# byungsook/neural-flow-style

Measured on AMD Instinct MI355X. Metric: stylization iters/sec on 200^3 smoke grid, 8 views, higher is better.
Workload: dtype f32 (3xbf16 split-limb MFMA, f32 accumulate)

## Files before the change

neural-flow-style_amd/_lib.py:

```python
from __future__ import annotations

import ctypes as C
import os
import subprocess

_HERE = os.path.dirname(os.path.abspath(__file__))
LIB_PATH = os.environ.get("NFS_LIB_PATH") or os.path.join(_HERE, "libnfs_hip.so")
CSRC_DIR = os.path.join(_HERE, "csrc")


class NfsLibraryError(RuntimeError):
    pass


NFS_EINVAL, NFS_ELAUNCH = -1, -2


class NfsError(RuntimeError):

    def __init__(self, name, code, msg):
        RuntimeError.__init__(self, "%s failed (%d): %s" % (name, code, msg))
        self.name, self.code = name, int(code)


# ... 111 lines not shown
    "nfs_gram_style_group_workspace_floats": [_P, _I],
    "nfs_gram_style_group_parts": [_P, _I],
    "nfs_gram_style_group_fwd": [_P, _I, _P, _P, _L, _P],
    "nfs_gram_group_bwd": [_P, _I, _P],
    "nfs_hist_loss_masked": [_P, _P, _P, _P, _P, _I, _I, _I, _I, _I, _F, _I, _P],
    "nfs_hist_loss_wide_workspace_floats": [_I, _I, _I, _I],
    "nfs_hist_loss_wide": [_P, _P, _P, _P, _P, _P, _L, _I, _I, _I, _I, _I, _F, _I, _P],
    "nfs_resize_bicubic_tf1": [_P, _P, _I, _I, _I, _I, _I, _I, _P],
    "nfs_style_mask_apply": [_P, _P, _P, _P, _I, _I, _I, _P],
    "nfs_style_mask_bwd": [_P, _P, _P, _P, _I, _I, _I, _P],
    "nfs_tv_loss": [_P, _P, _P, _I, _I, _I, _I, _F, _P],
    "nfs_p2g_fwd": [_P, _P, _P, _P, _P, _I, _I, C.POINTER(SplatCfg), _P],
    "nfs_p2g_bwd": [_P, _P, _P, _P, _P, _P, _P, _P, _I, _I, C.POINTER(SplatCfg), _P],
    "nfs_p2g_wavg_finish": [_P, _P, _P, _L, _I, _F, _P],
    "nfs_p2g_wavg_finish_bwd": [_P, _P, _P, _P, _P, _L, _I, _F, _P],
    "nfs_p2g_wavg_bwd": [_P, _P, _P, _P, _P, _P, _P, _I, _I, _F, C.POINTER(SplatCfg), _P],
    "nfs_g2p_fwd": [_P, _P, _P, _I, _I, _I, _I, _I, _L, _I, _P],
    "nfs_adam_tf_step": [_P, _P, _P, _P, _L, _F, _F, _F, _F, _P],
    "nfs_fill": [_P, _F, _L, _P],
    "nfs_axpy": [_P, _P, _F, _L, _P],
    "nfs_slab_pack": [_P, _P, _I, _L, _I, _I, _P],
    "nfs_colour_clamp_gather": [_P, _P, _P, _L, _I, _P],
    "nfs_clamp01_bwd": [_P, _P, _P, _L, _P],
    "nfs_colour_clamp_scatter_bwd": [_P, _P, _P, _P, _L, _I, _P],
    "nfs_iterate_update": [_P, _P, _L, _P],
}
_RESTYPE = {"nfs_last_error": C.c_char_p, "nfs_conv3x3_packed_floats": C.c_int64,
            "nfs_conv3x3_workspace_floats": C.c_int64, "nfs_gram_workspace_floats": C.c_int64,
            "nfs_conv3x3_relu_bits_words": C.c_int64, "nfs_gram_style_group_workspace_floats": C.c_int64, "nfs_hist_loss_wide_workspace_floats": C.c_int64,
            "nfs_conv3x3_executed_flops": C.c_double, "nfs_conv2d_packed_floats": C.c_int64,
            "nfs_conv2d_workspace_floats": C.c_int64, "nfs_conv2d_group_workspace_floats": C.c_int64}

_lib = None
ABI_VERSION = 152


def build(verbose=False):
    jobs = os.environ.get("MAX_JOBS") or str(min(os.cpu_count() or 4, 16))
    r = subprocess.run(["make", "-C", CSRC_DIR, "-j", jobs],
                       capture_output=True, text=True)
    if verbose or r.returncode != 0:
        print(r.stdout[-4000:], r.stderr[-4000:])
    if r.returncode != 0:
        raise NfsLibraryError("building libnfs_hip.so failed")
    return LIB_PATH


def lib():
    global _lib
    if _lib is None:
        if not os.path.exists(LIB_PATH):
            raise NfsLibraryError(
                "libnfs_hip.so is missing (%s): run `python -c 'import __graft_entry__ as g; g.build()'` "
                "-- there is no CPU fallback for the product path" % LIB_PATH)
        import torch
        try:
            L = C.CDLL(LIB_PATH)
        except OSError as e:
            raise NfsLibraryError("cannot load %s: %s" % (LIB_PATH, e))
        for name, argt in SIGNATURES.items():
            try:
                f = getattr(L, name)
            except AttributeError:
                raise NfsLibraryError("libnfs_hip.so does not export %s (stale build?)" % name)
            f.argtypes = argt
            f.restype = _RESTYPE.get(name, C.c_int)
        if L.nfs_version() < ABI_VERSION:
# ... 24 lines not shown
```

neural-flow-style_amd/csrc/api.hip:

```cpp
#include "common.h"

namespace nfs {
static thread_local char g_err[512] = "";
void set_error(const char* fmt, ...) {
  va_list ap;
  va_start(ap, fmt);
  vsnprintf(g_err, sizeof(g_err), fmt, ap);
  va_end(ap);
}
}

extern "C" {
int nfs_version(void) { return 152; }
const char* nfs_last_error(void) { return nfs::g_err; }
int nfs_device_cus(void) {
  int dev = 0;
  hipDeviceProp_t p;
  if (hipGetDevice(&dev) != hipSuccess || hipGetDeviceProperties(&p, dev) != hipSuccess) {
    nfs::set_error("nfs_device_cus: no HIP device");
    return NFS_ELAUNCH;
  }
  return p.multiProcessorCount;
}
}
```

neural-flow-style_amd/csrc/vgg.hip:

```cpp
#include "common.h"

#include <mutex>
#include <stdlib.h>

namespace nfs {

int64_t winograd_workspace_floats(int B, int H, int W, int K, int N);
int64_t winograd_packed_floats(int Ci, int Co);
int winograd_path(int B, int H, int W, int K, int N);
int winograd_tile();
int64_t winograd5_bits_words(int B, int H, int W, int C);
int winograd_pack(const float* w_hwio, float* up, int Ci, int Co, int kind, hipStream_t s);
int winograd_conv(const float* x, const float* U, const float* aux0, const float* aux1, float* y, float* ws, int B,
                  int H, int W, int K, int N, int mode, int relu, int cus, hipStream_t s, float* ypool,
                  const float* xmask, uint32_t* in_bits, uint32_t* out_bits, bool pooled_grad);
static inline bool winograd_eligible(int K, int N) {
  static const int min_ch = [] { const char* e = getenv("NFS_WINOGRAD_MIN_CH"); return e ? atoi(e) : 64; }();
  return K >= min_ch && N >= min_ch && K % 32 == 0 && N % 64 == 0;
}

typedef float f32x16 __attribute__((ext_vector_type(16)));

constexpr int KC = 32;
constexpr int LDS_STRIDE = 36;
constexpr int BM = 128;
constexpr int PATCH_MAX = 192;

struct ConvArgs {
  const float* x;
  const float* wp;
  const float* aux0;
  const float* aux1;
  float* y;
  float* ws;
  int B, H, W, Kc, Nc;
  int TH, TW, tiles_c;
  int relu, ksplit;
  int dbg;
};

template <int MODE>
__device__ __forceinline__ float conv_epilogue(const ConvArgs& a, float v, int n, int64_t idx) {
// ... 564 lines not shown
  return (int64_t)9 * Ci * Co + (winograd_eligible(K, N) ? winograd_packed_floats(Ci, Co) : 0);
}

int nfs_conv3x3_pack(const float* w_hwio, float* packed, int Ci, int Co, int kind, nfs_stream_t stream) {
  NFS_REQUIRE(w_hwio && packed, "nfs_conv3x3_pack: null pointer");
  NFS_REQUIRE(kind == 0 || kind == 1, "nfs_conv3x3_pack: kind must be 0 or 1");
  NFS_REQUIRE(Ci == 3 || (Ci % 64 == 0), "nfs_conv3x3_pack: Ci must be 3 or a multiple of 64");
  NFS_REQUIRE(Co % 64 == 0, "nfs_conv3x3_pack: Co must be a multiple of 64");
  const int64_t n = (int64_t)9 * Ci * Co;
  hipLaunchKernelGGL(pack_kernel, dim3(blocks_for(n, 256)), dim3(256), 0, as_stream(stream), w_hwio, packed, Ci, Co,
                     kind);
  const int K = kind == 0 ? Ci : Co, N = kind == 0 ? Co : Ci;
  if (winograd_eligible(K, N))
    if (int e = winograd_pack(w_hwio, packed + n, Ci, Co, kind, as_stream(stream))) return e;
  return check_launch("nfs_conv3x3_pack");
}

int64_t nfs_conv3x3_workspace_floats(int B, int H, int W, int Ci, int Co) {
  if (B <= 0 || H <= 0 || W <= 0 || Ci <= 0 || Co <= 0) return 0;
  if (winograd_eligible(Ci, Co) && winograd_eligible(Co, Ci) && H >= 2 && W >= 2)
    return winograd_workspace_floats(B, H, W, Ci > Co ? Ci : Co, Ci > Co ? Ci : Co);
  const int64_t n = Ci > Co ? Ci : Co;
  const int64_t want = (int64_t)16 * B * H * W * n;
  return want < ((int64_t)32 << 20) ? want : ((int64_t)32 << 20);
}

int64_t nfs_conv3x3_relu_bits_words(int B, int H, int W, int Ci, int Co, int pooled) {
  if (B <= 0 || H < 2 || W < 2 || Ci <= 0 || Co <= 0 || Ci % 64 || Co % 64) return 0;
  static const bool off = getenv("NFS_NO_RELU_BITS") != nullptr;
  ConvArgs a{nullptr, nullptr, nullptr, nullptr, nullptr, nullptr, B, H, W, Ci, Co, 0, 0, 0, 1, 1, 0};
  float dummy = 0.f;
  if (off || !takes_fused_pool(a, &dummy, INT64_MAX)) return 0;
  if (!pooled && winograd_path(B, H, W, Ci, Co) == 2) return winograd5_bits_words(B, H, W, Ci);
  const int64_t T = (int64_t)B * ((H + 3) / 4) * ((W + 3) / 4);
  return T * (Ci / 2) + (pooled ? T * (Co / 2) : 0);
}

double nfs_conv3x3_executed_flops(int B, int H, int W, int K, int N, int pooled) {
  if (B <= 0 || H <= 0 || W <= 0 || K <= 0 || N <= 0) return 0.0;
  static const bool no_wg = getenv("NFS_NO_WINOGRAD") != nullptr;
  const double direct = 2.0 * B * H * W * 9.0 * K * N;
  if (no_wg || !winograd_eligible(K, N) || H < 2 || W < 2) return direct;
  const int m = winograd_tile();
  if (m == 4 && !pooled && winograd_path(B, H, W, K, N) == 2)
    return 2.0 * 49.0 * B * ((H + 4) / 5) * ((W + 4) / 5) * (double)K * N;
  return 2.0 * (m + 2) * (m + 2) * B * ((H + m - 1) / m) * ((W + m - 1) / m) * (double)K * N;
}

static inline uint32_t* out_bits_of(uint32_t* relu_bits, int B, int H, int W, int Ci) {
  return relu_bits ? relu_bits + (int64_t)B * ((H + 3) / 4) * ((W + 3) / 4) * (Ci / 2) : nullptr;
}

int nfs_conv3x3_fwd(const float* x, const float* packed_fwd, const float* bias, float* y, int B, int H, int W, int Ci,
                    int Co, int relu, float* workspace, int64_t workspace_floats, uint32_t* relu_bits,
                    nfs_stream_t stream) {
  NFS_REQUIRE(x && packed_fwd && y, "nfs_conv3x3_fwd: null pointer");
  NFS_REQUIRE(B > 0 && H > 0 && W > 0, "nfs_conv3x3_fwd: non-positive dimension");
  NFS_REQUIRE((int64_t)B * H * W < ((int64_t)1 << 31) / 4, "nfs_conv3x3_fwd: too many pixels");
  NFS_REQUIRE(Co > 0 && Co % 64 == 0, "nfs_conv3x3_fwd: Co must be a multiple of 64");
  static const bool old_c3 = getenv("NFS_C3_OLD") != nullptr;
  if (Ci == 3 && Co == 64 && !old_c3) {
    const int tiles_x = (W + C3F_TW - 1) / C3F_TW, tiles_y = (H + C3F_TH - 1) / C3F_TH;
    static const int per_cu = [] { const char* e = getenv("NFS_C3F_BLOCKS"); return e ? atoi(e) : 4; }();
    const int64_t ntiles = (int64_t)B * tiles_x * tiles_y, cap = 256 * (int64_t)per_cu;
    hipLaunchKernelGGL(conv3x3_c3co64_fwd_kernel, dim3((unsigned)(per_cu > 0 && ntiles > cap ? cap : ntiles)), dim3(256), 0,
                       as_stream(stream), x, packed_fwd, bias, y, B, H, W, relu, tiles_x, tiles_y);
    return check_launch("nfs_conv3x3_fwd(c3, Co=64, MFMA)");
  }
  if (Ci == 3) {
    const int64_t n = (int64_t)B * H * W * (Co / 4);
    hipLaunchKernelGGL(conv3x3_c3_fwd_kernel, dim3(blocks_for(n, 256)), dim3(256), 27 * Co * sizeof(float),
                       as_stream(stream), x, packed_fwd, bias, y, B, H, W, Co, relu);
    return check_launch("nfs_conv3x3_fwd(c3)");
  }
  NFS_REQUIRE(Ci > 0 && Ci % 32 == 0, "nfs_conv3x3_fwd: Ci must be 3 or a multiple of 32");
  ConvArgs a{x, packed_fwd, bias, nullptr, y, nullptr, B, H, W, Ci, Co, 0, 0, 0, relu, 1, 0};
  return launch_conv<0>(a, workspace, workspace_floats, as_stream(stream), nullptr, nullptr, relu_bits, nullptr);
}

int nfs_conv3x3_dgrad(const float* gy, const float* packed_dgrad, const float* x_in, const float* addend, float* gx,
                      int B, int H, int W, int Ci, int Co, float* workspace, int64_t workspace_floats,
                      const uint32_t* relu_bits, int addend_unmasked, nfs_stream_t stream) {
  NFS_REQUIRE(gy && packed_dgrad && gx, "nfs_conv3x3_dgrad: null pointer");
  NFS_REQUIRE(B > 0 && H > 0 && W > 0, "nfs_conv3x3_dgrad: non-positive dimension");
  NFS_REQUIRE((int64_t)B * H * W < ((int64_t)1 << 31) / 4, "nfs_conv3x3_dgrad: too many pixels");
  NFS_REQUIRE(Co > 0 && Co % 32 == 0, "nfs_conv3x3_dgrad: Co must be a multiple of 32");
  if (Ci == 3) {
    NFS_REQUIRE(!x_in && !addend, "nfs_conv3x3_dgrad: Ci=3 takes no mask/addend");
    static const bool old_c3 = getenv("NFS_C3_OLD") != nullptr;
    if (Co == 64 && !old_c3) {
      const int tiles_x = (W + C3D_TW - 1) / C3D_TW, tiles_y = (H + C3D_TH - 1) / C3D_TH;
      static const int per_cu = [] { const char* e = getenv("NFS_C3D_BLOCKS"); return e ? atoi(e) : 2; }();
      const int64_t ntiles = (int64_t)B * tiles_x * tiles_y, cap = 256 * (int64_t)per_cu;
      hipLaunchKernelGGL(conv3x3_c3co64_dgrad_kernel, dim3((unsigned)(per_cu > 0 && ntiles > cap ? cap : ntiles)),
                         dim3(256), 0, as_stream(stream), gy, packed_dgrad, gx, B, H, W, tiles_x, tiles_y);
      return check_launch("nfs_conv3x3_dgrad(c3, Co=64, MFMA)");
    }
    const int64_t n = (int64_t)B * H * W;
    hipLaunchKernelGGL(conv3x3_c3_dgrad_kernel, dim3(blocks_for(n, 256)), dim3(256), 27 * Co * sizeof(float),
                       as_stream(stream), gy, packed_dgrad, gx, B, H, W, Co);
    return check_launch("nfs_conv3x3_dgrad(c3)");
  }
  NFS_REQUIRE(Ci > 0 && Ci % 64 == 0, "nfs_conv3x3_dgrad: Ci must be 3 or a multiple of 64");
  ConvArgs a{gy, packed_dgrad, x_in, addend, gx, nullptr, B, H, W, Co, Ci, 0, 0, 0, addend_unmasked ? 1 : 0, 1, 0};
  NFS_REQUIRE(!addend_unmasked || (x_in && takes_fused_pool(a, workspace, workspace_floats)),
              "nfs_conv3x3_dgrad: addend_unmasked needs x_in and the F(4x4) Winograd path");
  return launch_conv<1>(a, workspace, workspace_floats, as_stream(stream), nullptr, nullptr,
                        const_cast<uint32_t*>(relu_bits), nullptr);
}

int nfs_conv3x3_fwd_pool(const float* x, const float* packed_fwd, const float* bias, float* y, float* y_pool, int B, int H,
                         int W, int Ci, int Co, int relu, float* workspace, int64_t workspace_floats,
                         uint32_t* relu_bits, nfs_stream_t stream) {
  NFS_REQUIRE(x && packed_fwd && y_pool, "nfs_conv3x3_fwd_pool: null pointer");
  NFS_REQUIRE(B > 0 && H > 1 && W > 1, "nfs_conv3x3_fwd_pool: need H, W >= 2");
  NFS_REQUIRE((int64_t)B * H * W < ((int64_t)1 << 31) / 4, "nfs_conv3x3_fwd_pool: too many pixels");
  NFS_REQUIRE(Co > 0 && Co % 64 == 0 && Ci > 0 && Ci % 32 == 0, "nfs_conv3x3_fwd_pool: Ci %% 32, Co %% 64 required");
  ConvArgs a{x, packed_fwd, bias, nullptr, y, nullptr, B, H, W, Ci, Co, 0, 0, 0, relu, 1, 0};
  if (takes_fused_pool(a, workspace, workspace_floats)) {
    NFS_REQUIRE(y || relu_bits, "nfs_conv3x3_fwd_pool: without y the ReLU bit cache must be recorded");
    return launch_conv<0>(a, workspace, workspace_floats, as_stream(stream), y_pool, nullptr, relu_bits,
                          out_bits_of(relu_bits, B, H, W, Ci));
  }
  NFS_REQUIRE(!relu_bits, "nfs_conv3x3_fwd_pool: the ReLU bit cache needs the fused Winograd path "
                          "(nfs_conv3x3_relu_bits_words returned 0 for this layer)");
  NFS_REQUIRE(y, "nfs_conv3x3_fwd_pool: y may only be NULL on the fused Winograd path with a ReLU bit cache");
  if (int e = launch_conv<0>(a, workspace, workspace_floats, as_stream(stream))) return e;
  return nfs_avgpool2_fwd(y, y_pool, B, H, W, Co, stream);
}

int nfs_conv3x3_dgrad_pool(const float* gy_pool, const float* x_out, const float* packed_dgrad, const float* x_in,
                           const float* addend, float* gx, int B, int H, int W, int Ci, int Co, float* workspace,
                           int64_t workspace_floats, const uint32_t* relu_bits, int addend_unmasked,
                           nfs_stream_t stream) {
  NFS_REQUIRE(gy_pool && packed_dgrad && gx, "nfs_conv3x3_dgrad_pool: null pointer");
  NFS_REQUIRE(x_out || relu_bits, "nfs_conv3x3_dgrad_pool: x_out or the layer's ReLU bit cache is required");
  NFS_REQUIRE(B > 0 && H > 1 && W > 1, "nfs_conv3x3_dgrad_pool: need H, W >= 2");
  NFS_REQUIRE((int64_t)B * H * W < ((int64_t)1 << 31) / 4, "nfs_conv3x3_dgrad_pool: too many pixels");
  NFS_REQUIRE(Co > 0 && Co % 32 == 0 && Ci > 0 && Ci % 64 == 0, "nfs_conv3x3_dgrad_pool: Co %% 32, Ci %% 64 required");
  ConvArgs a{gy_pool, packed_dgrad, x_in, addend, gx, nullptr, B, H, W, Co, Ci, 0, 0, 0, addend_unmasked ? 1 : 0, 1, 0};
  NFS_REQUIRE(!addend_unmasked || (x_in && takes_fused_pool(a, workspace, workspace_floats)),
              "nfs_conv3x3_dgrad_pool: addend_unmasked needs x_in and the F(4x4) Winograd path");
  if (takes_fused_pool(a, workspace, workspace_floats)) {
    uint32_t* rb = const_cast<uint32_t*>(relu_bits);
    return launch_conv<1>(a, workspace, workspace_floats, as_stream(stream), nullptr, x_out, rb,
                          out_bits_of(rb, B, H, W, Ci), true);
  }
  NFS_REQUIRE(x_out, "nfs_conv3x3_dgrad_pool: x_out may only be NULL on the fused Winograd path");
  const int64_t n = (int64_t)B * H * W * Co;
  NFS_REQUIRE(workspace && workspace_floats >= n, "nfs_conv3x3_dgrad_pool: workspace of >= B*H*W*Co floats required");
  if (int e = nfs_avgpool2_bwd(gy_pool, x_out, nullptr, workspace, B, H, W, Co, stream)) return e;
  a.x = workspace;
  return launch_conv<1>(a, workspace + n, workspace_floats - n, as_stream(stream));
}

}
```

neural-flow-style_amd/csrc/winograd.hip:

```cpp
#include "common.h"
#include "winograd_math.h"
#include "winograd_gemm.h"

#include <algorithm>
#include <atomic>
#include <map>
#include <mutex>
#include <tuple>
#include <vector>

namespace nfs {

bool winograd_fusable(int K, int N);
bool winograd_fused_takes(int B, int H, int W, int K, int N);
int64_t winograd_fused_packed_floats(int K, int N);
int winograd_pack_fused(const float* up, float* uf, int K, int N, hipStream_t s);
int winograd_fused_conv(const float* x, const float* Uf, const float* aux0, const float* aux1, float* y, int B, int H,
                        int W, int K, int N, int mode, int relu, hipStream_t s, float* ypool, const float* xmask,
                        uint32_t* in_bits, uint32_t* out_bits, bool pooled_grad);

bool winograd5_channels(int K, int N);
bool winograd5_takes(int H, int W, int K, int N);
int64_t winograd5_packed_floats(int Ci, int Co);
int64_t winograd5_workspace_floats(int B, int H, int W, int K, int N);
int winograd5_pack(const float* w_hwio, float* up5, int Ci, int Co, int kind, hipStream_t s);
int64_t winograd5_bits_words(int B, int H, int W, int C);
int winograd5_conv(const float* x, const float* U5, const float* aux0, const float* aux1, float* y, float* ws, int B,
                   int H, int W, int K, int N, int mode, int relu, int cus, hipStream_t s, uint32_t* in_bits);

typedef float f32x16 __attribute__((ext_vector_type(16)));

__global__ void __launch_bounds__(256) winograd_pack_kernel(const float* __restrict__ w, float* __restrict__ up,
                                                            int Ci, int Co, int kind) {
  const int Kc = kind == 0 ? Ci : Co, Nc = kind == 0 ? Co : Ci;
  const int64_t gid = (int64_t)blockIdx.x * blockDim.x + threadIdx.x;
  if (gid >= (int64_t)Kc * Nc) return;
  const int n = (int)(gid % Nc), k = (int)(gid / Nc);
  float g[3][3];
#pragma unroll
  for (int r = 0; r < 3; ++r)
#pragma unroll
    for (int s = 0; s < 3; ++s) {
      if (kind == 0) g[r][s] = w[((int64_t)(r * 3 + s) * Ci + k) * Co + n];
      else g[r][s] = w[((int64_t)((2 - r) * 3 + (2 - s)) * Ci + n) * Co + k];
    }
  float t[4][3];
#pragma unroll
  for (int s = 0; s < 3; ++s) {
    t[0][s] = g[0][s];
    t[1][s] = 0.5f * (g[0][s] + g[1][s] + g[2][s]);
    t[2][s] = 0.5f * (g[0][s] - g[1][s] + g[2][s]);
    t[3][s] = g[2][s];
  }
#pragma unroll
  for (int r = 0; r < 4; ++r) {
    const float u[4] = {t[r][0], 0.5f * (t[r][0] + t[r][1] + t[r][2]), 0.5f * (t[r][0] - t[r][1] + t[r][2]), t[r][2]};
#pragma unroll
    for (int s = 0; s < 4; ++s) {
      const int comp = r * 4 + s;
      up[(((int64_t)comp * (Kc / 32) + k / 32) * Nc + n) * 32 + (k & 31)] = u[s];
    }
// ... 1511 lines not shown
  double flops = 0;
  for (int k = 0; k < n; ++k) {
    const int l = order[k];
    WgGemmArgs a{F[l], Dm[l], dF[l], (int64_t)HW[l], C[l], C[l], (int64_t)C[l] * C[l], 32, C[l], alpha[l], nullptr,
                 relu_mask[l] ? F[l] : nullptr};
    a.Uq16 = Dm[l];
    a.symb = 1;
    if (!gemm_rb16_applies(a) || C[l] % 64) return -1;
    a.mt = (int)((a.T + 79) / 80);
    a.nt = a.N / 64;
    a.Z = B;
    G.g[k] = a;
    G.ustart[k] = ub;
    ub += (a.mt * a.nt * a.Z + WG_XCDS - 1) / WG_XCDS * WG_XCDS;
    flops += 2.0 * B * (double)a.T * a.K * a.N;
  }
  G.ustart[n] = ub;
  launch_gemm_kernel<winograd_gemm_rb16_group_kernel<5, 1>>(G, gemm_lds_bytes<2, 80, 64, 0>(), ub,
                                                            GemmTimerRec{nullptr, nullptr, flops}, s);
  return check_launch("gram_bwd_gemm_group");
}

int winograd_tile() {
  static const int m = [] { const char* e = getenv("NFS_WINOGRAD_TILE"); return (e && atoi(e) == 2) ? 2 : 4; }();
  return m;
}

int winograd_path(int B, int H, int W, int K, int N) {
  if (winograd_tile() != 4) return 0;
  if (winograd_fusable(K, N) && winograd_fused_takes(B, H, W, K, N)) return 1;
  return winograd5_takes(H, W, K, N) ? 2 : 0;
}

int64_t winograd_workspace_floats(int B, int H, int W, int K, int N) {
  const int m = winograd_tile();
  const int64_t T = (int64_t)B * ((H + m - 1) / m) * ((W + m - 1) / m);
  const int64_t f4 = (m + 2) * (m + 2) * T * ((int64_t)K + (int64_t)N * winograd_ksplit(T, K)),
                f5 = m == 4 ? winograd5_workspace_floats(B, H, W, K, N) : 0;
  return f4 > f5 ? f4 : f5;
}

int64_t winograd_packed_floats(int Ci, int Co) {
  return (int64_t)(36 + 36 + 36 + 54) * Ci * Co + winograd_fused_packed_floats(Ci, Co) + winograd5_packed_floats(Ci, Co);
}

int winograd_pack(const float* w_hwio, float* up, int Ci, int Co, int kind, hipStream_t s) {
  const int64_t n = (int64_t)Ci * Co;
  if (winograd_tile() == 4) {
    hipLaunchKernelGGL(winograd_pack4_kernel, dim3(blocks_for(n, 256)), dim3(256), 0, s, w_hwio, up, Ci, Co, kind);
    const int Kc = kind == 0 ? Ci : Co, Nc = kind == 0 ? Co : Ci;
    hipLaunchKernelGGL(winograd_pack_frag_kernel, dim3(blocks_for(36 * n, 256)), dim3(256), 0, s, up, up + 36 * n, Kc, Nc,
                       36 * n);
    hipLaunchKernelGGL(winograd_pack_frag16_kernel, dim3(blocks_for(36 * n, 256)), dim3(256), 0, s, up, up + 72 * n, Kc,
                       Nc, 36 * n);
    if (winograd_fusable(Kc, Nc))
      if (int e = winograd_pack_fused(up, up + 108 * n, Kc, Nc, s)) return e;
    if (winograd5_channels(Kc, Nc))
      if (int e = winograd5_pack(w_hwio, up + 108 * n + winograd_fused_packed_floats(Ci, Co), Ci, Co, kind, s)) return e;
    winograd_pack_limbs16(up + 72 * n, up + 108 * n + winograd_fused_packed_floats(Ci, Co) + winograd5_packed_floats(Ci, Co),
                          Kc, Nc, 36, s);
  } else
    hipLaunchKernelGGL(winograd_pack_kernel, dim3(blocks_for(n, 256)), dim3(256), 0, s, w_hwio, up, Ci, Co, kind);
  return check_launch("winograd_pack");
}

int winograd_conv(const float* x, const float* U, const float* aux0, const float* aux1, float* y, float* ws, int B,
                  int H, int W, int K, int N, int mode, int relu, int cus, hipStream_t s, float* ypool,
                  const float* xmask, uint32_t* in_bits, uint32_t* out_bits, bool pooled_grad) {
  const int m = winograd_tile(), comps = (m + 2) * (m + 2);
  if (m == 4 && winograd_fusable(K, N) && winograd_fused_takes(B, H, W, K, N) && (!pooled_grad || mode == 1))
    return winograd_fused_conv(x, U + (int64_t)108 * K * N, aux0, aux1, y, B, H, W, K, N, mode, relu, s, ypool, xmask,
                               in_bits, out_bits, pooled_grad);
  if (m == 4 && !pooled_grad && !ypool && !out_bits && y && winograd5_takes(H, W, K, N))
    return winograd5_conv(x, U + (int64_t)108 * K * N + winograd_fused_packed_floats(K, N), aux0, aux1, y, ws, B, H, W, K, N,
                          mode, relu, cus, s, in_bits);
  const int TH = (H + m - 1) / m, TW = (W + m - 1) / m;
  const int64_t T = (int64_t)B * TH * TW;
  float* V = ws;
  float* M = ws + comps * T * K;
  const dim3 ig((blocks_for(T * (K / 2), 256) + 7) / 8 * 8);
  static const int64_t waves6_max = [] { const char* e = getenv("NFS_W4_WAVES6_MAX"); return e ? atoll(e) : (int64_t)65536; }();
  const bool in6 = m == 4 && K % 128 == 0 && T * K <= waves6_max, out6 = m == 4 && N % 128 == 0 && T * N <= waves6_max;
  const dim3 ig6((unsigned)((T * (K / 128) + 7) / 8 * 8));
  if (in6 && pooled_grad && mode == 1 && out_bits)
    hipLaunchKernelGGL(winograd_input4w_kernel<1>, ig6, dim3(64, 6), 0, s, x, V, B, H, W, K, TH, TW, out_bits);
  else if (in6 && !pooled_grad)
    hipLaunchKernelGGL(winograd_input4w_kernel<0>, ig6, dim3(64, 6), 0, s, x, V, B, H, W, K, TH, TW,
                       mode == 0 ? in_bits : (uint32_t*)nullptr);
  else
  if (m == 4 && pooled_grad && mode == 1 && out_bits)
    hipLaunchKernelGGL(winograd_input4_kernel<1>, ig, dim3(256), 0, s, x, V, B, H, W, K, TH, TW, xmask, out_bits);
  else if (m == 4 && pooled_grad)
    hipLaunchKernelGGL(winograd_input4_kernel<2>, ig, dim3(256), 0, s, x, V, B, H, W, K, TH, TW, xmask,
                       (uint32_t*)nullptr);
  else if (m == 4)
    hipLaunchKernelGGL(winograd_input4_kernel<0>, ig, dim3(256), 0, s, x, V, B, H, W, K, TH, TW,
                       (const float*)nullptr, mode == 0 ? in_bits : nullptr);
  else
    hipLaunchKernelGGL(winograd_input_kernel, dim3(blocks_for(T * (K / 4), 256)), dim3(256), 0, s, x, V, B, H, W, K, TH,
                       TW);
  WgGemmArgs a{V, U, M, T, K, N, (int64_t)K * N, (int64_t)N * 32, 32, 1.f, nullptr, nullptr};
  if (m == 4) {
    a.Uq = U + (int64_t)36 * K * N;
    a.Uq16 = U + (int64_t)72 * K * N;
    a.Ub16 = U + (int64_t)108 * K * N + winograd_fused_packed_floats(K, N) + winograd5_packed_floats(K, N);
  }
  const int nsplit = launch_batched_gemm(a, comps, cus, s);
  if (m == 4) {
// ... 114 lines not shown
```

neural-flow-style_amd/csrc/winograd5.hip:

```cpp
#include "common.h"
#include "winograd_gemm.h"

namespace nfs {

__device__ __forceinline__ void w5_g(const float g0, const float g1, const float g2, float* u) {
  u[0] = -0.5f * g0;
  u[1] = (-1.f / 3.f) * (g0 + g1 + g2);
  u[2] = (1.f / 9.f) * (g0 - g1 + g2);
  u[3] = (1.f / 36.f) * g0 + (1.f / 18.f) * g1 + (1.f / 9.f) * g2;
  u[4] = (-1.f / 60.f) * g0 + (1.f / 30.f) * g1 - (1.f / 15.f) * g2;
  u[5] = (32.f / 45.f) * g0 + (16.f / 45.f) * g1 + (8.f / 45.f) * g2;
  u[6] = g2;
}

__global__ void __launch_bounds__(256) winograd5_pack_kernel(const float* __restrict__ w, float* __restrict__ up, int Ci,
                                                             int Co, int kind) {
  const int Kc = kind == 0 ? Ci : Co, Nc = kind == 0 ? Co : Ci;
  const int64_t gid = (int64_t)blockIdx.x * blockDim.x + threadIdx.x;
  if (gid >= (int64_t)Kc * Nc) return;
  const int n = (int)(gid % Nc), k = (int)(gid / Nc);
  float g[3][3];
#pragma unroll
  for (int r = 0; r < 3; ++r)
#pragma unroll
// ... 8 lines not shown
    w5_g(g[0][s], g[1][s], g[2][s], u);
#pragma unroll
    for (int r = 0; r < 7; ++r) t[r][s] = u[r];
  }
#pragma unroll
  for (int r = 0; r < 7; ++r) {
    float u[7];
    w5_g(t[r][0], t[r][1], t[r][2], u);
#pragma unroll
    for (int q = 0; q < 7; ++q) up[(((int64_t)(r * 7 + q) * (Kc / 32) + k / 32) * Nc + n) * 32 + (k & 31)] = u[q];
  }
}

__device__ __forceinline__ void w5_bt(const float* d, float* o) {
#pragma clang fp contract(off)
  o[0] = -2.f * d[0] + 4.f * d[1] + 2.5f * d[2] - 5.f * d[3] - 0.5f * d[4] + d[5];
  o[1] = 2.f * d[1] - 2.f * d[2] - 4.5f * d[3] + 0.5f * d[4] + d[5];
  o[2] = -2.f * d[1] + 6.f * d[2] - 3.5f * d[3] - 1.5f * d[4] + d[5];
  o[3] = d[1] - 1.5f * d[2] - 2.f * d[3] + 1.5f * d[4] + d[5];
  o[4] = -d[1] + 2.5f * d[2] - 2.5f * d[4] + d[5];
  o[5] = 4.f * d[1] - 5.f * d[3] + d[5];
  o[6] = -2.f * d[1] + 4.f * d[2] + 2.5f * d[3] - 5.f * d[4] - 0.5f * d[5] + d[6];
}
__device__ __forceinline__ void w5_at(const float* m, float* o) {
#pragma clang fp contract(off)
  const float s12 = m[1] + m[2], d12 = m[1] - m[2], s34 = m[3] + m[4], d34 = m[3] - m[4];
  o[0] = m[0] + s12 + s34 + m[5];
  o[1] = d12 + 2.f * d34 + 0.5f * m[5];
  o[2] = s12 + 4.f * s34 + 0.25f * m[5];
  o[3] = d12 + 8.f * d34 + 0.125f * m[5];
  o[4] = s12 + 16.f * s34 + 0.0625f * m[5] + m[6];
}

__global__ void __launch_bounds__(256) winograd5_input_kernel(const float* __restrict__ x, float* __restrict__ V, int B,
                                                              int H, int W, int K, int TH, int TW,
                                                              uint32_t* __restrict__ bits) {
  const int64_t T = (int64_t)B * TH * TW;
  const unsigned per_xcd = gridDim.x / 8;
  const unsigned lb = (blockIdx.x % 8) * per_xcd + blockIdx.x / 8;
  const int64_t gid = (int64_t)lb * blockDim.x + threadIdx.x;
  if (gid >= T * K) return;
  const int c = (int)(gid % K);
  const int64_t tile = gid / K;
  const int tx = (int)(tile % TW), ty = (int)((tile / TW) % TH), b = (int)(tile / ((int64_t)TW * TH));
  const int y0 = 5 * ty - 1, x0 = 5 * tx - 1;
  float dv[7][7];
#pragma unroll
  for (int s = 0; s < 7; ++s)
#pragma unroll
    for (int r = 0; r < 7; ++r) {
      const int yc = min(max(y0 + r, 0), H - 1), xc = min(max(x0 + s, 0), W - 1);
      dv[s][r] = x[(((int64_t)b * H + yc) * W + xc) * K + c];
    }
  float t[7][7];
  unsigned long long mask = 0ull;
#pragma unroll
  for (int s = 0; s < 7; ++s) {
    float d[7];
    const int xx = x0 + s;
#pragma unroll
    for (int r = 0; r < 7; ++r) {
      const int yy = y0 + r;
      d[r] = (yy >= 0 && yy < H && xx >= 0 && xx < W) ? dv[s][r] : 0.f;
      if (r >= 1 && r <= 5 && s >= 1 && s <= 5)
        mask |= (unsigned long long)(d[r] > 0.f ? 1u : 0u) << (2 * ((r - 1) * 5 + (s - 1)));
    }
    w5_bt(d, t[s]);
  }
  if (bits) {
    const uint32_t lo = (uint32_t)mask, hi = (uint32_t)(mask >> 32);
    const uint32_t plo = __shfl_xor(lo, 1, 64), phi = __shfl_xor(hi, 1, 64);
    if (!(c & 1)) *reinterpret_cast<uint2*>(bits + gid) = make_uint2(lo | (plo << 1), hi | (phi << 1));
  }
  const int64_t comp_stride = T * K;
  float* vo = V + tile * K + c;
#pragma unroll
  for (int r = 0; r < 7; ++r) {
    const float row[7] = {t[0][r], t[1][r], t[2][r], t[3][r], t[4][r], t[5][r], t[6][r]};
    float o[7];
    w5_bt(row, o);
#pragma unroll
    for (int q = 0; q < 7; ++q) vo[(int64_t)(r * 7 + q) * comp_stride] = o[q];
  }
}

template <int MODE, int NSPLIT = 1>
__global__ void __launch_bounds__(256) winograd5_output_kernel(const float* __restrict__ M, const float* __restrict__ aux0,
                                                               const float* __restrict__ aux1, float* __restrict__ y,
                                                               int B, int H, int W, int N, int TH, int TW, int relu,
                                                               const uint32_t* __restrict__ bits) {
  const int64_t T = (int64_t)B * TH * TW;
  const int64_t gid = (int64_t)blockIdx.x * blockDim.x + threadIdx.x;
  if (gid >= T * N) return;
  const int c = (int)(gid % N);
  const int64_t tile = gid / N;
  const int tx = (int)(tile % TW), ty = (int)((tile / TW) % TH), b = (int)(tile / ((int64_t)TW * TH));
  const int64_t comp_stride = T * N;
  const float* mi = M + tile * N + c;
  float ad[5][5];
  if (MODE == 1) {
    const float* ap = aux1 ? aux1 : M;
#pragma unroll
// ... 16 lines not shown
    }
    w5_at(m, t[s]);
  }
  const float bias = (MODE == 0 && aux0) ? aux0[c] : 0.f;
  unsigned long long mask = 0ull;
  if (MODE == 1 && bits) {
    const uint2 mw = *reinterpret_cast<const uint2*>(bits + (gid & ~(int64_t)1));
    mask = (((unsigned long long)mw.y << 32) | mw.x) >> (c & 1);
  }
#pragma unroll
  for (int a = 0; a < 5; ++a) {
    const int yy = 5 * ty + a;
    if (yy >= H) continue;
    const float row[7] = {t[0][a], t[1][a], t[2][a], t[3][a], t[4][a], t[5][a], t[6][a]};
    float o[5];
    w5_at(row, o);
#pragma unroll
    for (int cc = 0; cc < 5; ++cc) {
      const int xx = 5 * tx + cc;
      if (xx >= W) continue;
      float v = o[cc];
      const int64_t idx = (((int64_t)b * H + yy) * W + xx) * N + c;
      if (MODE == 0) {
        v += bias;
        if (relu) v = fmaxf(v, 0.f);
      } else {
        const float adv = aux1 ? ad[a][cc] : 0.f;
        if (relu) v += adv;
        if (bits) v = ((mask >> (2 * (a * 5 + cc))) & 1ull) ? v : 0.f;
        else if (aux0) v = aux0[idx] > 0.f ? v : 0.f;
        if (!relu) v += adv;
      }
      y[idx] = v;
    }
  }
}

__global__ void __launch_bounds__(448) winograd5_input7_kernel(const float* __restrict__ x, float* __restrict__ V, int B,
                                                               int H, int W, int K, int TH, int TW,
                                                               uint32_t* __restrict__ bits) {
  __shared__ float tl[7][7][64];
  __shared__ unsigned long long mk[5][64];
  const int64_t T = (int64_t)B * TH * TW;
  const unsigned per_xcd = gridDim.x / 8;
  const unsigned lb = (blockIdx.x % 8) * per_xcd + blockIdx.x / 8;
  const int kg = K / 64;
  if ((int64_t)lb >= T * kg) return;
  const int64_t tile = lb / kg;
  const int lane = threadIdx.x, w = threadIdx.y, c = (int)(lb % kg) * 64 + lane;
  const int tx = (int)(tile % TW), ty = (int)((tile / TW) % TH), b = (int)(tile / ((int64_t)TW * TH));
  const int y0 = 5 * ty - 1, x0 = 5 * tx - 1;
  {
    const int xx = x0 + w, xc = min(max(xx, 0), W - 1);
    float d[7];
#pragma unroll
    for (int r = 0; r < 7; ++r) {
      const int yc = min(max(y0 + r, 0), H - 1);
      d[r] = x[(((int64_t)b * H + yc) * W + xc) * K + c];
    }
    unsigned long long mask = 0ull;
#pragma unroll
    for (int r = 0; r < 7; ++r) {
      const int yy = y0 + r;
      d[r] = (yy >= 0 && yy < H && xx >= 0 && xx < W) ? d[r] : 0.f;
      if (r >= 1 && r <= 5) mask |= (unsigned long long)(d[r] > 0.f ? 1u : 0u) << (2 * ((r - 1) * 5));
    }
// ... 63 lines not shown
  w5_at(row, o);
  const float bias = (MODE == 0 && aux0) ? aux0[c] : 0.f;
  const unsigned long long mask = ((((unsigned long long)mw.y << 32) | mw.x) >> (c & 1)) >> (2 * (a * 5));
#pragma unroll
  for (int cc = 0; cc < 5; ++cc) {
    const int xx = 5 * tx + cc;
    if (xx >= W) continue;
    float v = o[cc];
    const int64_t idx = (((int64_t)b * H + yy) * W + xx) * N + c;
    if (MODE == 0) {
      v += bias;
      if (relu) v = fmaxf(v, 0.f);
    } else {
      const float adv = aux1 ? ad[cc] : 0.f;
      if (relu) v += adv;
      if (bits) v = ((mask >> (2 * cc)) & 1ull) ? v : 0.f;
      else if (aux0) v = aux0[idx] > 0.f ? v : 0.f;
      if (!relu) v += adv;
    }
    y[idx] = v;
  }
}

bool winograd5_channels(int K, int N) {
  static const bool off = [] { const char* e = getenv("NFS_WG5"); return e && atoi(e) == 0; }();
  return !off && K >= 128 && N >= 128 && K % 64 == 0 && N % 64 == 0;
}
bool winograd5_takes(int H, int W, int K, int N) {
  if (!winograd5_channels(K, N) || H < 5 || W < 5) return false;
  const int64_t r5 = (int64_t)49 * ((H + 4) / 5) * ((W + 4) / 5), r4 = (int64_t)36 * ((H + 3) / 4) * ((W + 3) / 4);
  return r5 * 10 <= r4 * 9;
}

int64_t winograd5_packed_floats(int Ci, int Co) { return winograd5_channels(Ci, Co) ? (int64_t)98 * Ci * Co + (int64_t)147 * Ci * Co / 2 : 0; }

int64_t winograd5_workspace_floats(int B, int H, int W, int K, int N) {
  if (!winograd5_takes(H, W, K, N)) return 0;
  const int64_t T = (int64_t)B * ((H + 4) / 5) * ((W + 4) / 5);
  return (int64_t)49 * T * ((int64_t)K + (int64_t)N * winograd_ksplit(T, K));
}

int winograd5_pack(const float* w_hwio, float* up5, int Ci, int Co, int kind, hipStream_t s) {
  const int64_t n = (int64_t)Ci * Co;
  const int Kc = kind == 0 ? Ci : Co, Nc = kind == 0 ? Co : Ci;
  hipLaunchKernelGGL(winograd5_pack_kernel, dim3(blocks_for(n, 256)), dim3(256), 0, s, w_hwio, up5, Ci, Co, kind);
  winograd_pack_frag16(up5, up5 + 49 * n, Kc, Nc, 49 * n, s);
  winograd_pack_limbs16(up5 + 49 * n, up5 + 98 * n, Kc, Nc, 49, s);
  return check_launch("winograd5_pack");
}

int64_t winograd5_bits_words(int B, int H, int W, int C) { return (int64_t)B * ((H + 4) / 5) * ((W + 4) / 5) * C; }

int winograd5_conv(const float* x, const float* U5, const float* aux0, const float* aux1, float* y, float* ws, int B,
                   int H, int W, int K, int N, int mode, int relu, int cus, hipStream_t s, uint32_t* in_bits) {
  const int TH = (H + 4) / 5, TW = (W + 4) / 5;
  const int64_t T = (int64_t)B * TH * TW;
  float* V = ws;
  float* M = ws + 49 * T * K;
  static const int64_t waves7_max = [] { const char* e = getenv("NFS_W5_WAVES7_MAX"); return e ? atoll(e) : (int64_t)65536; }();
  if (T * K <= waves7_max) {
    const dim3 ig((unsigned)((T * (K / 64) + 7) / 8 * 8));
    hipLaunchKernelGGL(winograd5_input7_kernel, ig, dim3(64, 7), 0, s, x, V, B, H, W, K, TH, TW, mode == 0 ? in_bits : nullptr);
  } else {
    const dim3 ig((blocks_for(T * K, 256) + 7) / 8 * 8);
    hipLaunchKernelGGL(winograd5_input_kernel, ig, dim3(256), 0, s, x, V, B, H, W, K, TH, TW,
                       mode == 0 ? in_bits : nullptr);
  }
  WgGemmArgs a{V, U5, M, T, K, N, (int64_t)K * N, (int64_t)N * 32, 32, 1.f, nullptr, nullptr};
  a.Uq16 = U5 + (int64_t)49 * K * N;
  a.Ub16 = U5 + (int64_t)98 * K * N;
  const int nsplit = winograd_launch_batched_gemm(a, 49, cus, s);
  const unsigned ob = blocks_for(T * N, 256);
  if (nsplit != 1 && nsplit != 2) {
    set_error("winograd5_conv: unsupported number of K parts");
    return NFS_EINVAL;
  }
  const uint32_t* ib = aux0 ? in_bits : nullptr;
  if (T * N <= waves7_max) {
    const dim3 og((unsigned)(T * (N / 64)));
#define NFS_W5_OUT7(MODE_, NS_, BITS_)                                                                                \
    hipLaunchKernelGGL((winograd5_output7_kernel<MODE_, NS_>), og, dim3(64, 7), 0, s, M, aux0, aux1, y, B, H, W, N, TH, TW,  \
                       relu, BITS_)
    if (mode == 0 && nsplit == 1) NFS_W5_OUT7(0, 1, (const uint32_t*)nullptr);
    else if (mode == 0) NFS_W5_OUT7(0, 2, (const uint32_t*)nullptr);
    else if (nsplit == 1) NFS_W5_OUT7(1, 1, ib);
    else NFS_W5_OUT7(1, 2, ib);
#undef NFS_W5_OUT7
    return check_launch("winograd5_conv");
  }
  if (mode == 0 && nsplit == 1)
    hipLaunchKernelGGL((winograd5_output_kernel<0, 1>), dim3(ob), dim3(256), 0, s, M, aux0, aux1, y, B, H, W, N, TH, TW, relu,
                       (const uint32_t*)nullptr);
  else if (mode == 0)
    hipLaunchKernelGGL((winograd5_output_kernel<0, 2>), dim3(ob), dim3(256), 0, s, M, aux0, aux1, y, B, H, W, N, TH, TW, relu,
                       (const uint32_t*)nullptr);
  else if (nsplit == 1)
    hipLaunchKernelGGL((winograd5_output_kernel<1, 1>), dim3(ob), dim3(256), 0, s, M, aux0, aux1, y, B, H, W, N, TH, TW, relu, ib);
  else
    hipLaunchKernelGGL((winograd5_output_kernel<1, 2>), dim3(ob), dim3(256), 0, s, M, aux0, aux1, y, B, H, W, N, TH, TW, relu, ib);
  return check_launch("winograd5_conv");
}

}
```

Measured before the change: 445.6.

## Extend F(5x5) Winograd path to pooled conv layers with fused pool and mask

Routes pooled forward and pooled data-gradient 3x3 convs onto the F(5x5,3x3) Winograd path when the fused F(4x4) path does not apply and the layer is large. A new output kernel fuses bias, ReLU, ReLU-bit recording and 2x2 average pooling through shared memory. The input kernel gains templated variants that unpool the gradient and apply the ReLU mask from cached bits or a float mask. This cuts Winograd tile count for large pooled layers relative to F(4x4), and costs extra bit-cache layout logic plus new indexing paths that could misalign with existing buffers.

New measurement: 452.3, median of 6. +1.5%, better.

```diff
diff --git a/neural-flow-style_amd/_lib.py b/neural-flow-style_amd/_lib.py
--- a/neural-flow-style_amd/_lib.py
+++ b/neural-flow-style_amd/_lib.py
@@ -167,7 +167,7 @@
             "nfs_conv2d_workspace_floats": C.c_int64, "nfs_conv2d_group_workspace_floats": C.c_int64}
 
 _lib = None
-ABI_VERSION = 152
+ABI_VERSION = 153
 
 
 def build(verbose=False):
diff --git a/neural-flow-style_amd/csrc/api.hip b/neural-flow-style_amd/csrc/api.hip
--- a/neural-flow-style_amd/csrc/api.hip
+++ b/neural-flow-style_amd/csrc/api.hip
@@ -11,7 +11,7 @@
 }
 
 extern "C" {
-int nfs_version(void) { return 152; }
+int nfs_version(void) { return 153; }
 const char* nfs_last_error(void) { return nfs::g_err; }
 int nfs_device_cus(void) {
   int dev = 0;
diff --git a/neural-flow-style_amd/csrc/vgg.hip b/neural-flow-style_amd/csrc/vgg.hip
--- a/neural-flow-style_amd/csrc/vgg.hip
+++ b/neural-flow-style_amd/csrc/vgg.hip
@@ -8,6 +8,7 @@
 int64_t winograd_workspace_floats(int B, int H, int W, int K, int N);
 int64_t winograd_packed_floats(int Ci, int Co);
 int winograd_path(int B, int H, int W, int K, int N);
+int winograd_pooled_path(int B, int H, int W, int K, int N);
 int winograd_tile();
 int64_t winograd5_bits_words(int B, int H, int W, int C);
 int winograd_pack(const float* w_hwio, float* up, int Ci, int Co, int kind, hipStream_t s);
@@ -638,6 +639,8 @@
   float dummy = 0.f;
   if (off || !takes_fused_pool(a, &dummy, INT64_MAX)) return 0;
   if (!pooled && winograd_path(B, H, W, Ci, Co) == 2) return winograd5_bits_words(B, H, W, Ci);
+  if (pooled && winograd_pooled_path(B, H, W, Ci, Co) == 2)
+    return winograd5_bits_words(B, H, W, Ci) + winograd5_bits_words(B, H, W, Co);
   const int64_t T = (int64_t)B * ((H + 3) / 4) * ((W + 3) / 4);
   return T * (Ci / 2) + (pooled ? T * (Co / 2) : 0);
 }
@@ -648,13 +651,15 @@
   const double direct = 2.0 * B * H * W * 9.0 * K * N;
   if (no_wg || !winograd_eligible(K, N) || H < 2 || W < 2) return direct;
   const int m = winograd_tile();
-  if (m == 4 && !pooled && winograd_path(B, H, W, K, N) == 2)
+  if (m == 4 && (pooled ? winograd_pooled_path(B, H, W, K, N) : winograd_path(B, H, W, K, N)) == 2)
     return 2.0 * 49.0 * B * ((H + 4) / 5) * ((W + 4) / 5) * (double)K * N;
   return 2.0 * (m + 2) * (m + 2) * B * ((H + m - 1) / m) * ((W + m - 1) / m) * (double)K * N;
 }
 
-static inline uint32_t* out_bits_of(uint32_t* relu_bits, int B, int H, int W, int Ci) {
-  return relu_bits ? relu_bits + (int64_t)B * ((H + 3) / 4) * ((W + 3) / 4) * (Ci / 2) : nullptr;
+static inline uint32_t* out_bits_of(uint32_t* relu_bits, int B, int H, int W, int Ci, int Co) {
+  if (!relu_bits) return nullptr;
+  if (winograd_pooled_path(B, H, W, Ci, Co) == 2) return relu_bits + winograd5_bits_words(B, H, W, Ci);
+  return relu_bits + (int64_t)B * ((H + 3) / 4) * ((W + 3) / 4) * (Ci / 2);
 }
 
 int nfs_conv3x3_fwd(const float* x, const float* packed_fwd, const float* bias, float* y, int B, int H, int W, int Ci,
@@ -710,7 +715,7 @@
   NFS_REQUIRE(Ci > 0 && Ci % 64 == 0, "nfs_conv3x3_dgrad: Ci must be 3 or a multiple of 64");
   ConvArgs a{gy, packed_dgrad, x_in, addend, gx, nullptr, B, H, W, Co, Ci, 0, 0, 0, addend_unmasked ? 1 : 0, 1, 0};
   NFS_REQUIRE(!addend_unmasked || (x_in && takes_fused_pool(a, workspace, workspace_floats)),
-              "nfs_conv3x3_dgrad: addend_unmasked needs x_in and the F(4x4) Winograd path");
+              "nfs_conv3x3_dgrad: addend_unmasked needs x_in and the Winograd path");
   return launch_conv<1>(a, workspace, workspace_floats, as_stream(stream), nullptr, nullptr,
                         const_cast<uint32_t*>(relu_bits), nullptr);
 }
@@ -726,7 +731,7 @@
   if (takes_fused_pool(a, workspace, workspace_floats)) {
     NFS_REQUIRE(y || relu_bits, "nfs_conv3x3_fwd_pool: without y the ReLU bit cache must be recorded");
     return launch_conv<0>(a, workspace, workspace_floats, as_stream(stream), y_pool, nullptr, relu_bits,
-                          out_bits_of(relu_bits, B, H, W, Ci));
+                          out_bits_of(relu_bits, B, H, W, Ci, Co));
   }
   NFS_REQUIRE(!relu_bits, "nfs_conv3x3_fwd_pool: the ReLU bit cache needs the fused Winograd path "
                           "(nfs_conv3x3_relu_bits_words returned 0 for this layer)");
@@ -746,11 +751,11 @@
   NFS_REQUIRE(Co > 0 && Co % 32 == 0 && Ci > 0 && Ci % 64 == 0, "nfs_conv3x3_dgrad_pool: Co %% 32, Ci %% 64 required");
   ConvArgs a{gy_pool, packed_dgrad, x_in, addend, gx, nullptr, B, H, W, Co, Ci, 0, 0, 0, addend_unmasked ? 1 : 0, 1, 0};
   NFS_REQUIRE(!addend_unmasked || (x_in && takes_fused_pool(a, workspace, workspace_floats)),
-              "nfs_conv3x3_dgrad_pool: addend_unmasked needs x_in and the F(4x4) Winograd path");
+              "nfs_conv3x3_dgrad_pool: addend_unmasked needs x_in and the Winograd path");
   if (takes_fused_pool(a, workspace, workspace_floats)) {
     uint32_t* rb = const_cast<uint32_t*>(relu_bits);
     return launch_conv<1>(a, workspace, workspace_floats, as_stream(stream), nullptr, x_out, rb,
-                          out_bits_of(rb, B, H, W, Ci), true);
+                          out_bits_of(rb, B, H, W, Ci, Co), true);
   }
   NFS_REQUIRE(x_out, "nfs_conv3x3_dgrad_pool: x_out may only be NULL on the fused Winograd path");
   const int64_t n = (int64_t)B * H * W * Co;
diff --git a/neural-flow-style_amd/csrc/winograd.hip b/neural-flow-style_amd/csrc/winograd.hip
--- a/neural-flow-style_amd/csrc/winograd.hip
+++ b/neural-flow-style_amd/csrc/winograd.hip
@@ -26,7 +26,9 @@
 int winograd5_pack(const float* w_hwio, float* up5, int Ci, int Co, int kind, hipStream_t s);
 int64_t winograd5_bits_words(int B, int H, int W, int C);
 int winograd5_conv(const float* x, const float* U5, const float* aux0, const float* aux1, float* y, float* ws, int B,
-                   int H, int W, int K, int N, int mode, int relu, int cus, hipStream_t s, uint32_t* in_bits);
+                   int H, int W, int K, int N, int mode, int relu, int cus, hipStream_t s, uint32_t* in_bits,
+                   float* ypool, const float* xmask, uint32_t* out_bits, bool pooled_grad);
+bool winograd5_pooled_takes(int B, int H, int W, int K, int N);
 
 typedef float f32x16 __attribute__((ext_vector_type(16)));
 
@@ -1604,6 +1606,12 @@
   return winograd5_takes(H, W, K, N) ? 2 : 0;
 }
 
+int winograd_pooled_path(int B, int H, int W, int K, int N) {
+  if (winograd_tile() != 4) return 0;
+  if (winograd_fusable(K, N) && winograd_fused_takes(B, H, W, K, N)) return 1;
+  return winograd5_pooled_takes(B, H, W, K, N) ? 2 : 0;
+}
+
 int64_t winograd_workspace_floats(int B, int H, int W, int K, int N) {
   const int m = winograd_tile();
   const int64_t T = (int64_t)B * ((H + m - 1) / m) * ((W + m - 1) / m);
@@ -1643,9 +1651,10 @@
   if (m == 4 && winograd_fusable(K, N) && winograd_fused_takes(B, H, W, K, N) && (!pooled_grad || mode == 1))
     return winograd_fused_conv(x, U + (int64_t)108 * K * N, aux0, aux1, y, B, H, W, K, N, mode, relu, s, ypool, xmask,
                                in_bits, out_bits, pooled_grad);
-  if (m == 4 && !pooled_grad && !ypool && !out_bits && y && winograd5_takes(H, W, K, N))
+  const bool pooled = (mode == 0 && ypool) || (mode == 1 && pooled_grad);
+  if (m == 4 && (pooled ? winograd_pooled_path(B, H, W, K, N) == 2 : (!out_bits && y && winograd5_takes(H, W, K, N))))
     return winograd5_conv(x, U + (int64_t)108 * K * N + winograd_fused_packed_floats(K, N), aux0, aux1, y, ws, B, H, W, K, N,
-                          mode, relu, cus, s, in_bits);
+                          mode, relu, cus, s, in_bits, ypool, xmask, out_bits, pooled);
   const int TH = (H + m - 1) / m, TW = (W + m - 1) / m;
   const int64_t T = (int64_t)B * TH * TW;
   float* V = ws;
diff --git a/neural-flow-style_amd/csrc/winograd5.hip b/neural-flow-style_amd/csrc/winograd5.hip
--- a/neural-flow-style_amd/csrc/winograd5.hip
+++ b/neural-flow-style_amd/csrc/winograd5.hip
@@ -64,9 +64,11 @@
   o[4] = s12 + 16.f * s34 + 0.0625f * m[5] + m[6];
 }
 
+template <int POOLED>
 __global__ void __launch_bounds__(256) winograd5_input_kernel(const float* __restrict__ x, float* __restrict__ V, int B,
                                                               int H, int W, int K, int TH, int TW,
-                                                              uint32_t* __restrict__ bits) {
+                                                              uint32_t* __restrict__ bits,
+                                                              const float* __restrict__ xmask) {
   const int64_t T = (int64_t)B * TH * TW;
   const unsigned per_xcd = gridDim.x / 8;
   const unsigned lb = (blockIdx.x % 8) * per_xcd + blockIdx.x / 8;
@@ -76,13 +78,35 @@
   const int64_t tile = gid / K;
   const int tx = (int)(tile % TW), ty = (int)((tile / TW) % TH), b = (int)(tile / ((int64_t)TW * TH));
   const int y0 = 5 * ty - 1, x0 = 5 * tx - 1;
+  const int PH = H >> 1, PW = W >> 1;
+  [[maybe_unused]] unsigned long long nb[3][3];
+  if (POOLED == 1) {
+#pragma unroll
+    for (int dy = 0; dy < 3; ++dy)
+#pragma unroll
+      for (int dx = 0; dx < 3; ++dx) {
+        const int ny = min(max(ty + dy - 1, 0), TH - 1), nx = min(max(tx + dx - 1, 0), TW - 1);
+        const uint2 mw = *reinterpret_cast<const uint2*>(bits + (((int64_t)b * TH + ny) * TW + nx) * K + (c & ~1));
+        nb[dy][dx] = (((unsigned long long)mw.y << 32) | mw.x) >> (c & 1);
+      }
+  }
   float dv[7][7];
+  [[maybe_unused]] float mv[7][7];
 #pragma unroll
   for (int s = 0; s < 7; ++s)
 #pragma unroll
     for (int r = 0; r < 7; ++r) {
-      const int yc = min(max(y0 + r, 0), H - 1), xc = min(max(x0 + s, 0), W - 1);
-      dv[s][r] = x[(((int64_t)b * H + yc) * W + xc) * K + c];
+      if (!POOLED) {
+        const int yc = min(max(y0 + r, 0), H - 1), xc = min(max(x0 + s, 0), W - 1);
+        dv[s][r] = x[(((int64_t)b * H + yc) * W + xc) * K + c];
+      } else {
+        const int yc = min(max(y0 + r, 0) >> 1, PH - 1), xc = min(max(x0 + s, 0) >> 1, PW - 1);
+        dv[s][r] = x[(((int64_t)b * PH + yc) * PW + xc) * K + c];
+        if (POOLED == 2) {
+          const int ym = min(max(y0 + r, 0), H - 1), xm = min(max(x0 + s, 0), W - 1);
+          mv[s][r] = xmask[(((int64_t)b * H + ym) * W + xm) * K + c];
+        }
+      }
     }
   float t[7][7];
   unsigned long long mask = 0ull;
@@ -93,13 +117,26 @@
 #pragma unroll
     for (int r = 0; r < 7; ++r) {
       const int yy = y0 + r;
-      d[r] = (yy >= 0 && yy < H && xx >= 0 && xx < W) ? dv[s][r] : 0.f;
-      if (r >= 1 && r <= 5 && s >= 1 && s <= 5)
-        mask |= (unsigned long long)(d[r] > 0.f ? 1u : 0u) << (2 * ((r - 1) * 5 + (s - 1)));
+      if (!POOLED) {
+        d[r] = (yy >= 0 && yy < H && xx >= 0 && xx < W) ? dv[s][r] : 0.f;
+        if (r >= 1 && r <= 5 && s >= 1 && s <= 5)
+          mask |= (unsigned long long)(d[r] > 0.f ? 1u : 0u) << (2 * ((r - 1) * 5 + (s - 1)));
+      } else {
+        const bool ok = yy >= 0 && xx >= 0 && (yy >> 1) < PH && (xx >> 1) < PW;
+        bool m;
+        if (POOLED == 1) {
+          const int dy = r == 0 ? 0 : (r == 6 ? 2 : 1), ir = r == 0 ? 4 : (r == 6 ? 0 : r - 1);
+          const int dx = s == 0 ? 0 : (s == 6 ? 2 : 1), is = s == 0 ? 4 : (s == 6 ? 0 : s - 1);
+          m = (nb[dy][dx] >> (2 * (ir * 5 + is))) & 1ull;
+        } else {
+          m = mv[s][r] > 0.f;
+        }
+        d[r] = (ok && m) ? 0.25f * dv[s][r] : 0.f;
+      }
     }
     w5_bt(d, t[s]);
   }
-  if (bits) {
+  if (!POOLED && bits) {
     const uint32_t lo = (uint32_t)mask, hi = (uint32_t)(mask >> 32);
     const uint32_t plo = __shfl_xor(lo, 1, 64), phi = __shfl_xor(hi, 1, 64);
     if (!(c & 1)) *reinterpret_cast<uint2*>(bits + gid) = make_uint2(lo | (plo << 1), hi | (phi << 1));
@@ -182,6 +219,74 @@
         if (!relu) v += adv;
       }
       y[idx] = v;
+    }
+  }
+}
+
+template <int NSPLIT>
+__global__ void __launch_bounds__(256) winograd5_output_pool_kernel(const float* __restrict__ M, const float* __restrict__ bias_p,
+                                                                    float* __restrict__ y, float* __restrict__ ypool, int B,
+                                                                    int H, int W, int N, int TH, int TW, int relu,
+                                                                    uint32_t* __restrict__ bits) {
+  __shared__ float vs[10][10][64];
+  const int64_t T = (int64_t)B * TH * TW;
+  const int ng = N / 64, GH = (TH + 1) / 2, GW = (TW + 1) / 2;
+  const int64_t grp = blockIdx.x / ng;
+  const int lane = threadIdx.x & 63, q = threadIdx.x >> 6, c = (int)(blockIdx.x % ng) * 64 + lane;
+  const int gx = (int)(grp % GW), gy = (int)((grp / GW) % GH), b = (int)(grp / ((int64_t)GW * GH));
+  const int ty = 2 * gy + (q >> 1), tx = 2 * gx + (q & 1);
+  if (ty < TH && tx < TW) {
+    const int64_t tile = ((int64_t)b * TH + ty) * TW + tx, comp_stride = T * N, gid = tile * N + c;
+    const float* mi = M + gid;
+    float t[7][5];
+#pragma unroll
+    for (int s = 0; s < 7; ++s) {
+      float m[7];
+#pragma unroll
+      for (int r = 0; r < 7; ++r) {
+        m[r] = mi[(int64_t)(r * 7 + s) * comp_stride];
+#pragma unroll
+        for (int p = 1; p < NSPLIT; ++p) m[r] += mi[((int64_t)p * 49 + r * 7 + s) * comp_stride];
+      }
+      w5_at(m, t[s]);
+    }
+    const float bias = bias_p ? bias_p[c] : 0.f;
+    unsigned long long mask = 0ull;
+#pragma unroll
+    for (int a = 0; a < 5; ++a) {
+      const int yy = 5 * ty + a;
+      const float row[7] = {t[0][a], t[1][a], t[2][a], t[3][a], t[4][a], t[5][a], t[6][a]};
+      float o[5];
+      w5_at(row, o);
+#pragma unroll
+      for (int cc = 0; cc < 5; ++cc) {
+        const int xx = 5 * tx + cc;
+        float v = o[cc] + bias;
+        if (relu) v = fmaxf(v, 0.f);
+        vs[5 * (q >> 1) + a][5 * (q & 1) + cc][lane] = v;
+        if (yy < H && xx < W) {
+          mask |= (unsigned long long)(v > 0.f ? 1u : 0u) << (2 * (a * 5 + cc));
+          if (y) y[(((int64_t)b * H + yy) * W + xx) * N + c] = v;
+        }
+      }
+    }
+    if (bits) {
+      const uint32_t lo = (uint32_t)mask, hi = (uint32_t)(mask >> 32);
+      const uint32_t plo = __shfl_xor(lo, 1, 64), phi = __shfl_xor(hi, 1, 64);
+      if (!(c & 1)) *reinterpret_cast<uint2*>(bits + gid) = make_uint2(lo | (plo << 1), hi | (phi << 1));
+    }
+  }
+  __syncthreads();
+  const int PH = H >> 1, PW = W >> 1;
+  for (int k = q; k < 25; k += 4) {
+    const int pa = k / 5, pc = k % 5, py = 5 * gy + pa, px = 5 * gx + pc;
+    if (py < PH && px < PW) {
+      float p = 0.f;
+      p += vs[2 * pa][2 * pc][lane];
+      p += vs[2 * pa][2 * pc + 1][lane];
+      p += vs[2 * pa + 1][2 * pc][lane];
+      p += vs[2 * pa + 1][2 * pc + 1][lane];
+      ypool[(((int64_t)b * PH + py) * PW + px) * N + c] = 0.25f * p;
     }
   }
 }
@@ -311,6 +416,17 @@
   return r5 * 10 <= r4 * 9;
 }
 
+static int64_t waves7_max() {
+  static const int64_t v = [] { const char* e = getenv("NFS_W5_WAVES7_MAX"); return e ? atoll(e) : (int64_t)65536; }();
+  return v;
+}
+
+bool winograd5_pooled_takes(int B, int H, int W, int K, int N) {
+  if (!winograd5_takes(H, W, K, N)) return false;
+  const int64_t T = (int64_t)B * ((H + 4) / 5) * ((W + 4) / 5);
+  return T * (K < N ? K : N) > waves7_max();
+}
+
 int64_t winograd5_packed_floats(int Ci, int Co) { return winograd5_channels(Ci, Co) ? (int64_t)98 * Ci * Co + (int64_t)147 * Ci * Co / 2 : 0; }
 
 int64_t winograd5_workspace_floats(int B, int H, int W, int K, int N) {
@@ -331,19 +447,34 @@
 int64_t winograd5_bits_words(int B, int H, int W, int C) { return (int64_t)B * ((H + 4) / 5) * ((W + 4) / 5) * C; }
 
 int winograd5_conv(const float* x, const float* U5, const float* aux0, const float* aux1, float* y, float* ws, int B,
-                   int H, int W, int K, int N, int mode, int relu, int cus, hipStream_t s, uint32_t* in_bits) {
+                   int H, int W, int K, int N, int mode, int relu, int cus, hipStream_t s, uint32_t* in_bits,
+                   float* ypool, const float* xmask, uint32_t* out_bits, bool pooled_grad) {
   const int TH = (H + 4) / 5, TW = (W + 4) / 5;
   const int64_t T = (int64_t)B * TH * TW;
   float* V = ws;
   float* M = ws + 49 * T * K;
-  static const int64_t waves7_max = [] { const char* e = getenv("NFS_W5_WAVES7_MAX"); return e ? atoll(e) : (int64_t)65536; }();
-  if (T * K <= waves7_max) {
+  const bool pool_fwd = mode == 0 && ypool, pool_grad = mode == 1 && pooled_grad;
+  if ((pool_fwd || pool_grad) && !winograd5_pooled_takes(B, H, W, K, N)) {
+    set_error("winograd5_conv: the pooled forms need winograd5_pooled_takes");
+    return NFS_EINVAL;
+  }
+  if (pool_grad && !out_bits && !xmask) {
+    set_error("winograd5_conv: the pooled data gradient needs the output mask (bit cache or float)");
+    return NFS_EINVAL;
+  }
+  if (pool_grad) {
+    const dim3 ig((blocks_for(T * K, 256) + 7) / 8 * 8);
+    if (out_bits)
+      hipLaunchKernelGGL(winograd5_input_kernel<1>, ig, dim3(256), 0, s, x, V, B, H, W, K, TH, TW, out_bits, (const float*)nullptr);
+    else
+      hipLaunchKernelGGL(winograd5_input_kernel<2>, ig, dim3(256), 0, s, x, V, B, H, W, K, TH, TW, (uint32_t*)nullptr, xmask);
+  } else if (T * K <= waves7_max()) {
     const dim3 ig((unsigned)((T * (K / 64) + 7) / 8 * 8));
     hipLaunchKernelGGL(winograd5_input7_kernel, ig, dim3(64, 7), 0, s, x, V, B, H, W, K, TH, TW, mode == 0 ? in_bits : nullptr);
   } else {
     const dim3 ig((blocks_for(T * K, 256) + 7) / 8 * 8);
-    hipLaunchKernelGGL(winograd5_input_kernel, ig, dim3(256), 0, s, x, V, B, H, W, K, TH, TW,
-                       mode == 0 ? in_bits : nullptr);
+    hipLaunchKernelGGL(winograd5_input_kernel<0>, ig, dim3(256), 0, s, x, V, B, H, W, K, TH, TW,
+                       mode == 0 ? in_bits : nullptr, (const float*)nullptr);
   }
   WgGemmArgs a{V, U5, M, T, K, N, (int64_t)K * N, (int64_t)N * 32, 32, 1.f, nullptr, nullptr};
   a.Uq16 = U5 + (int64_t)49 * K * N;
@@ -354,8 +485,16 @@
     set_error("winograd5_conv: unsupported number of K parts");
     return NFS_EINVAL;
   }
+  if (pool_fwd) {
+    const dim3 og((unsigned)((int64_t)B * ((TH + 1) / 2) * ((TW + 1) / 2) * (N / 64)));
+    if (nsplit == 1)
+      hipLaunchKernelGGL(winograd5_output_pool_kernel<1>, og, dim3(256), 0, s, M, aux0, y, ypool, B, H, W, N, TH, TW, relu, out_bits);
+    else
+      hipLaunchKernelGGL(winograd5_output_pool_kernel<2>, og, dim3(256), 0, s, M, aux0, y, ypool, B, H, W, N, TH, TW, relu, out_bits);
+    return check_launch("winograd5_conv(pool)");
+  }
   const uint32_t* ib = aux0 ? in_bits : nullptr;
-  if (T * N <= waves7_max) {
+  if (T * N <= waves7_max()) {
     const dim3 og((unsigned)(T * (N / 64)));
 #define NFS_W5_OUT7(MODE_, NS_, BITS_)                                                                                \
     hipLaunchKernelGGL((winograd5_output7_kernel<MODE_, NS_>), og, dim3(64, 7), 0, s, M, aux0, aux1, y, B, H, W, N, TH, TW,  \
```
